# zixunh/vipe

Measured on AMD Instinct MI355X. Metric: dense-BA+flow update iters/s, 512x384 48-KF graph, higher is better.
Workload: dtype f16 (correlation, GRU; fp32 accumulate) + f32 geometry/BA (fp64 reduced system)

## Files before the change

### include/vipe_amd.h

```cpp
#ifndef VIPE_AMD_H
#define VIPE_AMD_H

#include <stdint.h>

#ifdef __cplusplus
extern "C" {
#endif

#define VIPE_F16 0
#define VIPE_F32 1
#define VIPE_F64 2
#define VIPE_U8 3

#define VIPE_OK 0
#define VIPE_EINVAL (-1)
#define VIPE_ENOSPACE (-2)
#define VIPE_EUNSUPPORTED (-3)

#define VIPE_PYRAMID_REFERENCE 0
#define VIPE_PYRAMID_BLOCKED 1

#define VIPE_CAM_PINHOLE 0
#define VIPE_CAM_MEI 1
#define VIPE_CAM_PANORAMA 2
// ... 225 lines not shown
                                 int64_t Lv, int heads, int C, int L, int64_t Lq, int P, int dtype, void* stream);

#define VIPE_ACT_NONE 0
#define VIPE_ACT_RELU 1
#define VIPE_ACT_SIGMOID 2
#define VIPE_ACT_TANH 3
int vipe_conv_pack_weights(const void* d_w_oihw, void* d_w_packed, int Cout, int Cin, int KH, int KW, int src_dtype,
                           void* stream);
int vipe_conv2d_nhwc_f16(const void* d_x, const void* d_w_packed, const float* d_bias, const float* d_extra,
                         void* d_y, int B, int H, int W, int Cin, int cin_total, int cin_off, int Cout,
                         int cout_total, int cout_off, int KH, int KW, int act, void* stream);

int vipe_conv_packed_dims(int Cout, int Cin, int KH, int KW, int* cout_pad, int* cin_pad, int* k_pad);

#define VIPE_CONV_PARTIAL 6
#define VIPE_CONV_ACCINIT_F32 0x100
int vipe_conv2d_fused(const void* d_x0, int x0_ctot, int x0_coff, const void* d_x1, int x1_ctot, int x1_coff,
                      int split, const void* d_w_packed, const float* d_bias, const float* d_extra, int extra_stride,
                      int extra_off, void* d_y, int y_ctot, int y_coff, void* d_y2, int y2_ctot, int y2_coff,
                      const void* d_net, int net_ctot, int net_coff, const void* d_z, float* d_fout,
                      const void* d_accinit, int ai_ctot, int ai_coff, int B, int H, int W, int Cin, int Cout, int KH,
                      int KW, int act, int mode, void* stream);

typedef struct {
  const void *corr0_w, *corr2_w, *flow0_w, *flow2_w, *gw_w, *zr_w, *q_w, *zr_s_w, *q_s_w, *heads0_w, *heads2_w, *agg2_w, *eta_w;
  const void *zr_n_w, *zr_x_w;
  const float *corr0_b, *corr2_b, *flow0_b, *flow2_b, *gw_b, *zr_b, *q_b, *heads0_b, *heads2_b, *agg2_b, *eta_b;
  const float* glo_wT;
  const float* glo_b;
} vipe_update_weights;
typedef struct {
  int E, H, W, n_src;
  const void* levels[4];
  const float* coords;
  const int* slots;
  int h2, w2, pyramid_layout;
  const void* corr;
  const void* motn;
  const void* net;
  void* net_out;
  void* xbuf;
  const void* pgate;
  void *c1, *f1, *zb, *rnet;
  void* hbuf;
  float* dw;
  float *glo, *extra;
  const int *order, *rowptr;
  void *agg, *a2;
  float* eta;
  void* side_stream;
  float* pzr;
  int gate_state;
} vipe_update_buffers;
int vipe_update_operator(const vipe_update_weights* weights, const vipe_update_buffers* buffers, void* stream);

int vipe_update_gate_state(const vipe_update_weights* weights, const vipe_update_buffers* buffers, const void* d_net,
                           int parts, void* stream);
typedef struct {
  const vipe_update_weights* weights;
  const vipe_update_buffers* buffers;
  const void* net;
  const int* bounds;
  int n_bounds;
} vipe_gate_state_job;
int vipe_update_gate_state_piece(void* user, int piece, int n_pieces, void* stream);

int vipe_glo_context(const float* d_glo_sum, const float* d_wT, const float* d_bias, float* d_extra, int E, int hw,
// ... 93 lines not shown
```

### vipe_amd/csrc/conv_mfma.hip

```cpp
#include <stdlib.h>

#include <type_traits>

#include "common.cuh"

namespace {

typedef _Float16 half8 __attribute__((ext_vector_type(8)));
typedef _Float16 half4 __attribute__((ext_vector_type(4)));
typedef float float16v __attribute__((ext_vector_type(16)));
typedef float float4v __attribute__((ext_vector_type(4)));

enum Epi { EPI_PLAIN = 0, EPI_GLO = 1, EPI_ZR = 2, EPI_Q = 3, EPI_HEADS = 4, EPI_ETA = 5, EPI_PARTIAL = 6 };

struct ConvArgs {
  const half_t* x0; int x0_ctot, x0_coff;
  const half_t* x1; int x1_ctot, x1_coff;
  int split;
  const half_t* w;
  const float* bias;
  const float* extra;
  int extra_stride, extra_off;
  half_t* y; int y_ctot, y_coff;
  int B, H, W, Cin, Cin_pad, Cout, Cout_pad, KH, KW, nsteps;
  int act, epi;
  const half_t* net; int net_ctot, net_coff;
  const half_t* zbuf;
  half_t* y2; int y2_ctot, y2_coff;
  float* fout;
  const half_t* accinit; int ai_ctot, ai_coff;
  int ai_f32;
  int f_wp, f_hwp, f_tiles, f_pieces, f_xbytes, f_p1lo, f_p1hi;
  unsigned f_magic;
};

constexpr int BNP = 128;
constexpr int BK = 64;

__device__ __forceinline__ int swz(int row, int k8) { return row * 128 + ((k8 ^ ((row >> 1) & 7)) << 4); }

__device__ __forceinline__ float act_apply(float v, int act) {
  switch (act) {
    case VIPE_ACT_RELU: return fmaxf(v, 0.0f);
    case VIPE_ACT_SIGMOID: return 1.0f / (1.0f + __expf(-v));
    case VIPE_ACT_TANH: return tanhf(v);
    default: return v;
// ... 316 lines not shown

constexpr int H32_PIECES = (HALO_ROWS + 15) / 16;
constexpr int H32_XBYTES = H32_PIECES * 1024;
constexpr int H32_XP = (H32_PIECES + 7) / 8;
constexpr int H32_BK = 32;

__device__ __forceinline__ int swzf(int row) { return ((row >> 2) & 1) << 1; }
__device__ __forceinline__ int swz32(int row, int c) { return row * 64 + ((c ^ swzf(row)) << 4); }


__device__ __forceinline__ int flat_pixel(int q, int e, int H, int W, int wp, int hwp, unsigned magic) {
  if ((unsigned)q >= (unsigned)hwp) return -1;
  const int y = (int)__umulhi((unsigned)q, magic);
  const int x = q - y * wp;
  return x < W ? (e * H + y) * W + x : -1;
}

template <int BMC, int KS, bool M16, int VAR = 0, bool FLAT = false>
__global__ __launch_bounds__(512) __attribute__((amdgpu_waves_per_eu(4, 4))) void conv_halo32_kernel(ConvArgs a, int gy) {
  static_assert(M16, "only the 16x16x32 form exists");
  constexpr int MI = BMC >= 128 ? 4 : 2, NJ = BMC == 32 ? 2 : 4;
  constexpr int BP = HALO_TH * HALO_TW;
  constexpr int WSTAGE = BMC * 64;
  extern __shared__ __align__(16) unsigned char lds[];

  const int tid = threadIdx.x, lane = tid & 63, wave = __builtin_amdgcn_readfirstlane(tid >> 6);
  const int wm = BMC == 32 ? 0 : (wave >> 2), wn = wave & 3;
  const int pxh = BMC == 32 ? (wave >> 2) * 32 : 0;
  const int L = xcd_remap(blockIdx.x, gridDim.x);
  const int tile = L / gy, cout0 = (L % gy) * BMC;
// ... 207 lines not shown
#pragma unroll
        for (int j = 0; j < NJ; ++j) {
          const int64_t m = pix_of(wn * 64 + j * 16 + l16);
          if (FLAT && m < 0) continue;
#pragma unroll
          for (int i = 0; i < MI; ++i) {
            const int cg = cout0 + wm * (MI * 16) + i * 16 + 4 * lk;
            if (cg + 4 <= a.Cout)
              *reinterpret_cast<float4*>(a.fout + m * a.y_ctot + a.y_coff + cg) =
                  make_float4(acc16[i][j][0], acc16[i][j][1], acc16[i][j][2], acc16[i][j][3]);
          }
        }
        return;
      }
    }
    constexpr int PITCH = BMC + 8;
    half_t* stage = reinterpret_cast<half_t*>(lds);
    auto stage_all = [&](auto ACTC) {
      constexpr int ACT = decltype(ACTC)::value;
      auto put = [&](int cl, int pl, float4 b, float v0, float v1, float v2, float v3) {
        half4 h;
        h[0] = (half_t)act_apply(v0 + b.x, ACT);
        h[1] = (half_t)act_apply(v1 + b.y, ACT);
        h[2] = (half_t)act_apply(v2 + b.z, ACT);
        h[3] = (half_t)act_apply(v3 + b.w, ACT);
        *reinterpret_cast<half4*>(stage + pl * PITCH + cl) = h;
      };
      auto bias4 = [&](int cl) {
        const int cg = cout0 + cl;
        float4 b = *reinterpret_cast<const float4*>(a.bias + cg);
// ... 477 lines not shown
  VIPE_CHECK_ARG(d_w_oihw && d_w_packed);
  VIPE_CHECK_ARG(src_dtype == VIPE_F16 || src_dtype == VIPE_F32);
  int cp, cinp, kp;
  if (vipe_conv_packed_dims(Cout, Cin, KH, KW, &cp, &cinp, &kp) != VIPE_OK) return VIPE_EINVAL;
  VIPE_CHECK_ARG(Cin == 4 || Cin % 8 == 0);
  const int64_t total = (int64_t)kp * cp;
  pack_weights_kernel<<<(int)std::min<int64_t>((total + 255) / 256, 4096), 256, 0, as_stream(stream)>>>(
      d_w_oihw, (half_t*)d_w_packed, Cout, Cin, KH, KW, cp, cinp, kp, src_dtype == VIPE_F32, Cin == 4);
  return vipe_launch_status();
}

}

namespace {

template <typename K>
void allow_lds(K kernel, std::atomic<uint64_t>& seen, size_t bytes) {
  vipe_once_per_device(seen, [&] { (void)hipFuncSetAttribute((const void*)kernel, hipFuncAttributeMaxDynamicSharedMemorySize, (int)bytes); });
}
constexpr size_t MAX_LDS = 160 * 1024;

bool flat_geometry(ConvArgs& a, int pad) {
  a.f_wp = a.W + pad;
  a.f_hwp = a.H * a.f_wp;
  a.f_tiles = (a.f_hwp + 255) / 256;
  a.f_magic = (unsigned)(((1ull << 32) + (unsigned)a.f_wp - 1) / (unsigned)a.f_wp);
  const int rows = 256 + 2 * a.f_wp + 2;
  a.f_pieces = (rows + 15) / 16;
  a.f_xbytes = a.f_pieces * 1024;
  a.f_p1lo = (a.f_wp + 1) / 16;
  a.f_p1hi = (a.f_wp + 256) / 16;
  return a.f_wp >= 2 && a.f_pieces <= 8 * H32_XP && a.f_hwp < (1 << 23);
}

inline bool needs_tile_kernel(const ConvArgs& a) { return a.accinit || a.epi == EPI_PARTIAL || a.ai_f32; }

template <int BMC, int KS, int VAR, bool FLAT>
int launch_halo32(const ConvArgs& a, int tiles, int gy, size_t lds, hipStream_t s) {
  static std::atomic<uint64_t> seen{0};
  allow_lds(conv_halo32_kernel<BMC, KS, true, VAR, FLAT>, seen, FLAT ? MAX_LDS : lds);
  conv_halo32_kernel<BMC, KS, true, VAR, FLAT><<<dim3(tiles * gy), 512, lds, s>>>(a, gy);
  return vipe_launch_status();
}

template <bool FLAT>
int launch_halo_family(ConvArgs& a, int cp, int64_t M, hipStream_t s) {
  const bool split_ok = a.split >= a.Cin || a.split % H32_BK == 0;
  const int tiles = FLAT ? a.B * a.f_tiles : (int)(M / (HALO_TH * HALO_TW));
  const size_t xb = FLAT ? (size_t)a.f_xbytes : (size_t)H32_XBYTES;
  if (needs_tile_kernel(a)) {
    const bool ok = cp >= 64 && split_ok && !(a.KH == 3 && a.Cout <= 16) && !(a.epi == EPI_PARTIAL && a.Cout % 4 != 0) &&
                    !(a.ai_f32 && !a.accinit);
    if (!ok) return VIPE_EUNSUPPORTED;
  }
  if (a.KH == 3 && a.Cout <= 16 && cp == 32 && split_ok && (a.epi == EPI_HEADS || a.epi == EPI_ETA || a.epi == EPI_PLAIN)) {
    static std::atomic<uint64_t> seen{0};
    const size_t lds = 2 * NRW_WBYTES + 2 * xb + 1024;
    allow_lds(conv_halo32_narrow_kernel<FLAT>, seen, FLAT ? MAX_LDS : lds);
    conv_halo32_narrow_kernel<FLAT><<<dim3(tiles), 512, lds, s>>>(a);
    return vipe_launch_status();
  }
  if (!split_ok) return VIPE_EUNSUPPORTED;
  const int bmc = cp >= 128 ? 128 : cp;
  const int gy = cp >= 128 ? cp / 128 : 1;
// ... 119 lines not shown
                                  int y_coff, void* d_y2, int y2_ctot, int y2_coff, const void* d_net, int net_ctot,
                                  int net_coff, const void* d_z, float* d_fout, const void* d_accinit, int ai_ctot,
                                  int ai_coff, int B, int H, int W, int Cin, int Cout, int KH, int KW, int act, int mode,
                                  void* stream) {
  VIPE_CHECK_ARG(d_x0 && d_w_packed && d_bias);
  VIPE_CHECK_ARG(!d_accinit || (ai_ctot % 4 == 0 && ai_coff % 4 == 0 && ai_coff + Cout <= ai_ctot));
  VIPE_CHECK_ARG(B >= 0 && H > 0 && W > 0 && Cin > 0 && Cout > 0 && (KH & 1) && (KW & 1));
  if (Cin == 4) {
    VIPE_CHECK_ARG(split >= Cin && x0_ctot % 4 == 0 && x0_coff % 4 == 0);
  } else {
    VIPE_CHECK_ARG(Cin % 8 == 0 && x0_ctot % 8 == 0 && x0_coff % 8 == 0);
    VIPE_CHECK_ARG(split >= Cin || (split % 64 == 0 && d_x1 && x1_ctot % 8 == 0 && x1_coff % 8 == 0));
  }
  const int ai_f32 = (mode & VIPE_CONV_ACCINIT_F32) != 0;
  mode &= ~VIPE_CONV_ACCINIT_F32;
  VIPE_CHECK_ARG(mode >= EPI_PLAIN && mode <= EPI_PARTIAL);
  if (mode == EPI_PARTIAL) VIPE_CHECK_ARG(d_fout && y_ctot % 4 == 0 && y_coff % 4 == 0 && y_coff + Cout <= y_ctot && !d_extra);
  if (mode == EPI_PLAIN) VIPE_CHECK_ARG(d_y && y_ctot % 4 == 0 && y_coff % 4 == 0);
  if (mode == EPI_GLO) VIPE_CHECK_ARG(d_net && d_fout);
  if (mode == EPI_ZR) VIPE_CHECK_ARG(d_y && d_y2 && d_net && Cout == 256);
  if (mode == EPI_Q) VIPE_CHECK_ARG(d_y && d_net && d_z && Cout == 128);
  if (mode == EPI_HEADS) VIPE_CHECK_ARG(d_fout && Cout == 4);
  if (mode == EPI_ETA) VIPE_CHECK_ARG(d_fout && Cout == 1);
  ConvArgs a = {};
  a.x0 = (const half_t*)d_x0; a.x0_ctot = x0_ctot; a.x0_coff = x0_coff;
  a.x1 = (const half_t*)(d_x1 ? d_x1 : d_x0); a.x1_ctot = d_x1 ? x1_ctot : x0_ctot; a.x1_coff = d_x1 ? x1_coff : x0_coff;
  a.split = split > Cin ? Cin : split;
  a.w = (const half_t*)d_w_packed; a.bias = d_bias; a.extra = d_extra; a.extra_stride = extra_stride; a.extra_off = extra_off;
  a.y = (half_t*)d_y; a.y_ctot = y_ctot; a.y_coff = y_coff;
  a.y2 = (half_t*)d_y2; a.y2_ctot = y2_ctot; a.y2_coff = y2_coff;
  a.net = (const half_t*)d_net; a.net_ctot = net_ctot; a.net_coff = net_coff;
  a.zbuf = (const half_t*)d_z; a.fout = d_fout;
  a.accinit = (const half_t*)d_accinit; a.ai_ctot = ai_ctot; a.ai_coff = ai_coff; a.ai_f32 = ai_f32;
  a.B = B; a.H = H; a.W = W; a.Cin = Cin; a.Cout = Cout; a.KH = KH; a.KW = KW;
  a.act = act; a.epi = mode;
  return launch_conv(a, as_stream(stream));
}

}
```

### vipe_amd/csrc/update_op.hip

```cpp
#include "common.cuh"

namespace {

__global__ __launch_bounds__(384) void glo_gemm_kernel(const float* __restrict__ glo, const float* __restrict__ wT ,
                                                       const float* __restrict__ b, float* __restrict__ extra, float inv_hw) {
  __shared__ float g[128];
  const int e = blockIdx.x, t = threadIdx.x;
  if (t < 128) g[t] = glo[(int64_t)e * 128 + t] * inv_hw;
  __syncthreads();
  float acc = b[t];
#pragma unroll 8
  for (int k = 0; k < 128; ++k) acc = __builtin_fmaf(g[k], wT[k * 384 + t], acc);
  extra[(int64_t)e * 384 + t] = acc;
}

__global__ __launch_bounds__(256) void update_finish_kernel(const float* __restrict__ coords1, const float* __restrict__ dw,
                                                            const unsigned char* __restrict__ mask, float* __restrict__ target,
                                                            float* __restrict__ weight, const float* __restrict__ eta,
                                                            const int64_t* __restrict__ du, float* __restrict__ damping,
                                                            int64_t n_px, int64_t n_eta, int P) {
  const int64_t i = (int64_t)blockIdx.x * 256 + threadIdx.x;
  if (i < n_px) {
    const float2 c = reinterpret_cast<const float2*>(coords1)[i];
    const float4 d = reinterpret_cast<const float4*>(dw)[i];
// ... 84 lines not shown
                          nullptr, 0, 0, b->net, 128, 0, b->zb, nullptr, b->pgate, 384, 256, E, H, W, 320, 128, 3, 3,
                          VIPE_ACT_NONE, 3, stream));
  } else if (b->pgate) {
    RUN(vipe_conv2d_fused(b->net, 128, 0, b->xbuf, 320, 128, 128, wt->zr_s_w, wt->zr_b, b->extra, 384, 0, b->zb, 128, 0, b->rnet,
                          128, 0, b->net, 128, 0, nullptr, nullptr, b->pgate, 384, 0, E, H, W, 320, 256, 3, 3, VIPE_ACT_NONE, 2,
                          stream));
    RUN(vipe_conv2d_fused(b->rnet, 128, 0, b->xbuf, 320, 128, 128, wt->q_s_w, wt->q_b, b->extra, 384, 256, b->net_out, 128, 0,
                          nullptr, 0, 0, b->net, 128, 0, b->zb, nullptr, b->pgate, 384, 256, E, H, W, 320, 128, 3, 3,
                          VIPE_ACT_NONE, 3, stream));
  } else {
    RUN(vipe_conv2d_fused(b->net, 128, 0, b->xbuf, 320, 0, 128, wt->zr_w, wt->zr_b, b->extra, 384, 0, b->zb, 128, 0, b->rnet, 128,
                          0, b->net, 128, 0, nullptr, nullptr, nullptr, 0, 0, E, H, W, 448, 256, 3, 3, VIPE_ACT_NONE, 2, stream));
    RUN(vipe_conv2d_fused(b->rnet, 128, 0, b->xbuf, 320, 0, 128, wt->q_w, wt->q_b, b->extra, 384, 256, b->net_out, 128, 0, nullptr,
                          0, 0, b->net, 128, 0, b->zb, nullptr, nullptr, 0, 0, E, H, W, 448, 128, 3, 3, VIPE_ACT_NONE, 3, stream));
  }
  RUN(vipe_conv2d_fused(b->net_out, 128, 0, nullptr, 0, 0, 128, wt->heads0_w, wt->heads0_b, nullptr, 0, 0, b->hbuf, 384, 0,
                        nullptr, 0, 0, nullptr, 0, 0, nullptr, nullptr, nullptr, 0, 0, E, H, W, 128, 384, 3, 3, VIPE_ACT_RELU, 0,
                        stream));
  const bool two_tails = s2 && b->n_src > 0;
  if (two_tails) FORK(2);
  RUN(vipe_conv2d_fused(b->hbuf, 384, 0, nullptr, 0, 0, 256, wt->heads2_w, wt->heads2_b, nullptr, 0, 0, nullptr, 0, 0, nullptr, 0,
                        0, nullptr, 0, 0, nullptr, b->dw, nullptr, 0, 0, E, H, W, 256, 4, 3, 3, VIPE_ACT_NONE, 4,
                        two_tails ? stream2 : stream));
  if (b->n_src > 0) {
    VIPE_CHECK_ARG(b->order && b->rowptr && b->agg && b->a2 && b->eta);
    RUN(vipe_segment_mean_nhwc_f16(b->hbuf, 384, 256, b->order, b->rowptr, b->agg, b->n_src, (int64_t)H * W, 128, stream));
    RUN(vipe_conv2d_fused(b->agg, 128, 0, nullptr, 0, 0, 128, wt->agg2_w, wt->agg2_b, nullptr, 0, 0, b->a2, 128, 0, nullptr, 0, 0,
                          nullptr, 0, 0, nullptr, nullptr, nullptr, 0, 0, b->n_src, H, W, 128, 128, 3, 3, VIPE_ACT_RELU, 0,
                          stream));
    RUN(vipe_conv2d_fused(b->a2, 128, 0, nullptr, 0, 0, 128, wt->eta_w, wt->eta_b, nullptr, 0, 0, nullptr, 0, 0, nullptr, 0, 0,
                          nullptr, 0, 0, nullptr, b->eta, nullptr, 0, 0, b->n_src, H, W, 128, 1, 3, 3, VIPE_ACT_NONE, 5, stream));
  }
  if (two_tails) JOIN(3);
#undef FORK
#undef JOIN
#undef RUN
  return vipe_launch_status();
}

VIPE_EXPORT int vipe_update_gate_state(const vipe_update_weights* wt, const vipe_update_buffers* b, const void* d_net,
                                       int parts, void* stream) {
  VIPE_CHECK_ARG(wt && b && b->E >= 0 && b->H > 0 && b->W > 0 && parts >= 1 && parts <= 3);
  if (b->E == 0) return VIPE_OK;
  VIPE_CHECK_ARG(d_net && (!(parts & 1) || (b->glo && b->extra)) && (!(parts & 2) || (b->pgate && b->pzr && wt->zr_n_w)));
  const int E = b->E, H = b->H, W = b->W;
  hipStream_t s = as_stream(stream);
// ... 62 lines not shown
```

### vipe_amd/slam/update_engine.py

```python

import ctypes
import os

import torch

from .._lib import check, lib, parse_struct, ptr, stream_ptr

UpdateWeights = parse_struct("vipe_update_weights")
UpdateBuffers = parse_struct("vipe_update_buffers")
GateStateJob = parse_struct("vipe_gate_state_job")

ACT = {"none": 0, "relu": 1, "sigmoid": 2, "tanh": 3}
EPI = {"plain": 0, "glo": 1, "zr": 2, "q": 3, "heads": 4, "eta": 5, "partial": 6}
ACCINIT_F32 = 0x100
CORR_CH = 200


class _Packed:

    def __init__(self, w_oihw, bias, device):
        w = w_oihw.detach().to(device=device, dtype=torch.float16).contiguous()
        self.cout, self.cin, self.kh, self.kw = w.shape
        cp, cinp, kp = ctypes.c_int(), ctypes.c_int(), ctypes.c_int()
        check(lib().vipe_conv_packed_dims(self.cout, self.cin, self.kh, self.kw, ctypes.addressof(cp),
                                          ctypes.addressof(cinp), ctypes.addressof(kp)), "conv_packed_dims")
        self.packed = torch.empty(kp.value * cp.value, dtype=torch.float16, device=device)
        check(lib().vipe_conv_pack_weights(ptr(w), ptr(self.packed), self.cout, self.cin, self.kh, self.kw, 0,
                                           stream_ptr(w)), "conv_pack_weights")
        assert bias.numel() == self.cout, (tuple(bias.shape), self.cout)
        self.bias = torch.zeros(cp.value, dtype=torch.float32, device=device)
        self.bias[:self.cout] = bias.detach().to(device=device, dtype=torch.float32).reshape(-1)
        self.flops_per_pixel = 2.0 * self.cout * self.cin * self.kh * self.kw


def segment_csr(ix, n_src):
    order = torch.argsort(ix, stable=True).to(torch.int32).contiguous()
    counts = torch.bincount(ix, minlength=n_src)
    rowptr = torch.zeros(n_src + 1, dtype=torch.int32, device=ix.device)
    rowptr[1:] = torch.cumsum(counts, 0).to(torch.int32)
    return order, rowptr


class UpdateEngine:
    def __init__(self, module, device):
        self.device = device
        self.m = module
        self._bufs = {}
# ... 19 lines not shown
        wz, bz = wb(m.gru.convz)
        wr, br = wb(m.gru.convr)
        self.zr = _Packed(torch.cat([wz, wr], 0), torch.cat([bz, br], 0), d)
        wq, bq = wb(m.gru.convq)
        self.q = _Packed(wq, bq, d)
        rest = list(range(0, 128)) + list(range(256, 448))
        self.zr_s = _Packed(torch.cat([wz, wr], 0)[:, rest].contiguous(), torch.cat([bz, br], 0), d)
        self.q_s = _Packed(wq[:, rest].contiguous(), bq, d)
        self.gates_inp = _Packed(torch.cat([wz, wr, wq], 0)[:, 128:256].contiguous(), torch.zeros(384, device=d), d)
        self.zr_n = _Packed(torch.cat([wz, wr], 0)[:, 0:128].contiguous(), torch.cat([bz, br], 0), d)
        self.zr_x = _Packed(torch.cat([wz, wr], 0)[:, 256:448].contiguous(), torch.cat([bz, br], 0), d)
        wd0, bd0 = wb(m.delta[0])
        ww0, bw0 = wb(m.weight[0])
        wa1, ba1 = wb(m.agg.conv1)
        self.heads0 = _Packed(torch.cat([wd0, ww0, wa1], 0), torch.cat([bd0, bw0, ba1], 0), d)
        wd2, bd2 = wb(m.delta[2])
        ww2, bw2 = wb(m.weight[2])
        h2 = torch.zeros(4, 256, 3, 3, device=d, dtype=f16)
        h2[0:2, 0:128] = wd2[:2]
        h2[2:4, 128:256] = ww2[:2]
        self.heads2 = _Packed(h2, torch.cat([bd2[:2], bw2[:2]], 0), d)
        self.agg2 = _Packed(*wb(m.agg.conv2), d)
        self.eta = _Packed(*wb(m.agg.eta[0]), d)
        self.upmask = _Packed(*wb(m.agg.upmask[0]), d)
        g = m.gru
        self.glo_w = torch.cat([g.convz_glo.weight, g.convr_glo.weight, g.convq_glo.weight], 0).detach().to(d).float() \
            .reshape(384, 128).t().contiguous()
        self.glo_b = torch.cat([g.convz_glo.bias, g.convr_glo.bias, g.convq_glo.bias], 0).detach().to(d).float()
        wd_ = UpdateWeights()
        for name, pk in dict(corr0=self.corr0, corr2=self.corr2, flow0=self.flow0, flow2=self.flow2, gw=self.gw, zr=self.zr,
                             q=self.q, heads0=self.heads0, heads2=self.heads2, agg2=self.agg2, eta=self.eta).items():
            setattr(wd_, name + "_w", pk.packed.data_ptr())
            setattr(wd_, name + "_b", pk.bias.data_ptr())
        wd_.zr_s_w, wd_.q_s_w = self.zr_s.packed.data_ptr(), self.q_s.packed.data_ptr()
        wd_.zr_n_w, wd_.zr_x_w = self.zr_n.packed.data_ptr(), self.zr_x.packed.data_ptr()
        wd_.glo_wT, wd_.glo_b = self.glo_w.data_ptr(), self.glo_b.data_ptr()
        self._wdesc = wd_
        self._bdesc = {}

    def _conv(self, pk, x0, x0_coff, B, H, W, y=None, y_coff=0, act="none", mode="plain", x1=None, x1_coff=0,
              split=None, extra=None, extra_off=0, y2=None, y2_coff=0, net=None, net_coff=0, z=None, fout=None,
              cin=None, accinit=None, ai_coff=0):
        cin = pk.cin if cin is None else cin
        split = cin if split is None else split
        check(lib().vipe_conv2d_fused(
            ptr(x0), x0.shape[-1], x0_coff, ptr(x1), x1.shape[-1] if x1 is not None else 0, x1_coff, split,
            ptr(pk.packed), ptr(pk.bias), ptr(extra), extra.shape[-1] if extra is not None else 0, extra_off,
            ptr(y), (y if y is not None else fout).shape[-1] if (y is not None or mode == "partial") else 0, y_coff,
            ptr(y2), y2.shape[-1] if y2 is not None else 0, y2_coff,
            ptr(net), net.shape[-1] if net is not None else 0, net_coff, ptr(z), ptr(fout), ptr(accinit),
            accinit.shape[-1] if accinit is not None else 0, ai_coff, B, H, W, cin, pk.cout,
# ... 56 lines not shown
            cum, acc = [0], 0.0
            for f in fractions[:-1]:
                acc += f
                cum.append(min(E, int(round(E * acc / sum(fractions)))))
            cum.append(E)
            bounds = (ctypes.c_int * len(cum))(*cum)
            job.bounds, job.n_bounds = ctypes.addressof(bounds), len(cum)
        fn = ctypes.cast(lib().vipe_update_gate_state_piece, ctypes.c_void_p).value
        gs = dict(net_ptr=net.data_ptr(), pgate_ptr=pgate.data_ptr(), shape=tuple(net.shape), pzr=pzr, extra=extra,
                  n_staged=E, keep=(b, job, bounds), gen=self._gate_gen)
        return gs, (lambda stream: (stream.cuda_stream, fn, ctypes.addressof(job)))

    def gate_state_matches(self, gs, net, pgate):
        return (gs is not None and pgate is not None and gs["net_ptr"] == net.data_ptr() and
                gs["pgate_ptr"] == pgate.data_ptr() and gs["shape"] == tuple(net.shape) and gs.get("gen") == self._gate_gen)

    def _buf(self, name, shape, dtype=torch.float16):
        t = self._bufs.get(name)
        if t is None or tuple(t.shape) != tuple(shape) or t.dtype != dtype:
            t = torch.empty(shape, dtype=dtype, device=self.device)
            self._bufs[name] = t
        return t

    @torch.no_grad()
    def forward_nhwc(self, net, xbuf, corr, motn, ix=None, n_src=None, net_out=None, want_upmask=False, csr=None,
                     pgate=None, native=True, gate_state=None):
        E, H, W, _ = net.shape
        if not self.gate_state_matches(gate_state, net, pgate):
            gate_state = None
        if gate_state is None:
# ... 32 lines not shown
                       accinit=gate_state["pzr"], ai_coff=0, cin=192)
            if Es < E:
                self._conv(self.zr_s, net[Es:], 0, E - Es, H, W, x1=xbuf[Es:], x1_coff=128, split=128, y=zb[Es:], y2=rnet[Es:],
                           net=net[Es:], mode="zr", extra=extra[Es:], accinit=pgate[Es:], ai_coff=0)
            self._conv(self.q_s, rnet, 0, E, H, W, x1=xbuf, x1_coff=128, split=128, y=net_out, net=net, z=zb, mode="q",
                       extra=extra, extra_off=256, accinit=pgate, ai_coff=256)
        elif pgate is not None:
            self._conv(self.zr_s, net, 0, E, H, W, x1=xbuf, x1_coff=128, split=128, y=zb, y2=rnet, net=net, mode="zr",
                       extra=extra, accinit=pgate, ai_coff=0)
            self._conv(self.q_s, rnet, 0, E, H, W, x1=xbuf, x1_coff=128, split=128, y=net_out, net=net, z=zb, mode="q",
                       extra=extra, extra_off=256, accinit=pgate, ai_coff=256)
        else:
            self._conv(self.zr, net, 0, E, H, W, x1=xbuf, split=128, y=zb, y2=rnet, net=net, mode="zr", extra=extra)
            self._conv(self.q, rnet, 0, E, H, W, x1=xbuf, split=128, y=net_out, net=net, z=zb, mode="q", extra=extra,
                       extra_off=256)
        self._conv(self.heads0, net_out, 0, E, H, W, y=hbuf, act="relu")
        self._conv(self.heads2, hbuf, 0, E, H, W, mode="heads", fout=dw, cin=256)
        eta = upmask = None
        if ix is not None:
            if n_src is None:
                n_src = int(ix.max().item()) + 1 if ix.numel() else 0
            if csr is None:
                csr = segment_csr(ix, n_src)
            order, rowptr = csr
            agg = self._buf("agg", (n_src, H, W, 128))
            check(lib().vipe_segment_mean_nhwc_f16(ptr(hbuf), 384, 256, ptr(order), ptr(rowptr), ptr(agg), n_src, H * W,
                                                   128, stream_ptr(hbuf)), "segment_mean")
            a2 = self._buf("a2", (n_src, H, W, 128))
            eta = self._buf("eta", (n_src, H, W), torch.float32)
            self._conv(self.agg2, agg, 0, n_src, H, W, y=a2, act="relu")
            self._conv(self.eta, a2, 0, n_src, H, W, mode="eta", fout=eta)
            if want_upmask:
                upmask = torch.empty((n_src, H, W, 576), dtype=torch.float16, device=self.device)
                self._conv(self.upmask, a2, 0, n_src, H, W, y=upmask)
        return net_out, dw, eta, upmask

    def _forward_native(self, net, xbuf, corr, motn, ix, n_src, net_out, want_upmask, csr, pgate, scratch,
                        gate_state=None):
        c1, f1, zb, rnet, hbuf, dw, glo = scratch
        E, H, W, _ = net.shape
        extra = self._buf("extra", (E, 384), torch.float32)
        eta = agg = a2 = order = rowptr = None
        if ix is not None:
            if n_src is None:
                n_src = int(ix.max().item()) + 1 if ix.numel() else 0
            if csr is None:
                csr = segment_csr(ix, n_src)
            order, rowptr = csr
            agg = self._buf("agg", (n_src, H, W, 128))
            a2 = self._buf("a2", (n_src, H, W, 128))
            eta = self._buf("eta", (n_src, H, W), torch.float32)
        lookup = isinstance(corr, tuple)
        tensors = (net, net_out, xbuf, motn, pgate, c1, f1, zb, rnet, hbuf, dw, glo, extra, order, rowptr, agg, a2, eta) + \
            ((tuple(corr[1]) + (corr[2],) + ((corr[3],) if len(corr) > 3 and corr[3] is not None else ())) if lookup else (corr,))
        pzr = gate_state["pzr"] if gate_state is not None else None
        two_streams = E >= self.op_side_min_edges
        if two_streams and self._op_side is None:
            self._op_side = torch.cuda.Stream(device=self.device)
        key = tuple(0 if t is None else t.data_ptr() for t in tensors) + (E, H, W, n_src or 0, two_streams,
                                                                         0 if pzr is None else pzr.data_ptr(),
                                                                         0 if pzr is None else int(gate_state["n_staged"]))
        b = self._bdesc.get(key)
        if b is None:
            if len(self._bdesc) > 16:
                self._bdesc.clear()
            b = UpdateBuffers()
            b.E, b.H, b.W, b.n_src = E, H, W, int(n_src or 0) if ix is not None else 0
            if lookup:
                lv = corr[1]
                for i in range(4):
                    b.levels[i] = lv[i].data_ptr()
                b.coords = corr[2].data_ptr()
                b.slots = corr[3].data_ptr() if len(corr) > 3 and corr[3] is not None else None
                if len(corr) > 4 and corr[4] is not None:
                    b.h2, b.w2 = int(corr[4][0]), int(corr[4][1])
                else:
                    b.h2, b.w2 = int(lv[2].shape[3]) << 2, int(lv[2].shape[4]) << 2
                b.pyramid_layout = 1 if lv[0].dim() == 7 else 0
            else:
                b.corr = corr.data_ptr()
            for name, t in dict(motn=motn, net=net, net_out=net_out, xbuf=xbuf, pgate=pgate, c1=c1, f1=f1, zb=zb, rnet=rnet,
                                hbuf=hbuf, dw=dw, glo=glo, extra=extra, order=order, rowptr=rowptr, agg=agg, a2=a2,
                                eta=eta).items():
                setattr(b, name, None if t is None else t.data_ptr())
            if pzr is not None:
                b.pzr, b.gate_state = pzr.data_ptr(), int(gate_state["n_staged"])
            if two_streams:
                b.side_stream = self._op_side.cuda_stream
            self._bdesc[key] = b
        check(lib().vipe_update_operator(ctypes.addressof(self._wdesc), ctypes.addressof(b), stream_ptr(net)),
              "update_operator")
        upmask = None
        if want_upmask and ix is not None:
            upmask = torch.empty((n_src, H, W, 576), dtype=torch.float16, device=self.device)
            self._conv(self.upmask, a2, 0, n_src, H, W, y=upmask)
        return net_out, dw, eta, upmask

    @torch.no_grad()
# ... 28 lines not shown
```

Measured before the change: 263.0.

## Fuse heads 3x3 conv into heads0 epilogue and split agg branch per consumer

Splits the heads0 conv by consumer. The agg1 slice is computed first so the aggregation chain can fork onto the side stream early. The delta/weight 256-channel slice now runs a new fused epilogue: it applies the 4-output heads2 3x3 conv in registers and LDS via MFMA, writes interior pixels directly, and writes halo contributions to a border buffer. A small finish kernel adds neighbour-tile border sums, bias and sigmoid. This removes the hbuf round-trip and a separate heads2 launch, at the cost of extra LDS use, an extra kernel and a more complex epilogue.

```diff
diff --git a/include/vipe_amd.h b/include/vipe_amd.h
--- a/include/vipe_amd.h
+++ b/include/vipe_amd.h
@@ -263,6 +263,7 @@
 int vipe_conv_packed_dims(int Cout, int Cin, int KH, int KW, int* cout_pad, int* cin_pad, int* k_pad);
 
 #define VIPE_CONV_PARTIAL 6
+#define VIPE_CONV_HEADS_FUSED 7
 #define VIPE_CONV_ACCINIT_F32 0x100
 int vipe_conv2d_fused(const void* d_x0, int x0_ctot, int x0_coff, const void* d_x1, int x1_ctot, int x1_coff,
                       int split, const void* d_w_packed, const float* d_bias, const float* d_extra, int extra_stride,
@@ -271,12 +272,19 @@
                       const void* d_accinit, int ai_ctot, int ai_coff, int B, int H, int W, int Cin, int Cout, int KH,
                       int KW, int act, int mode, void* stream);
 
+int vipe_heads_fused_ok(int H, int W);
+int vipe_heads_border_floats(int E, int H, int W, int64_t* n_floats);
+int vipe_heads_finish(float* d_dw, const float* d_border, const float* d_bias, int E, int H, int W, void* stream);
+
 typedef struct {
   const void *corr0_w, *corr2_w, *flow0_w, *flow2_w, *gw_w, *zr_w, *q_w, *zr_s_w, *q_s_w, *heads0_w, *heads2_w, *agg2_w, *eta_w;
   const void *zr_n_w, *zr_x_w;
   const float *corr0_b, *corr2_b, *flow0_b, *flow2_b, *gw_b, *zr_b, *q_b, *heads0_b, *heads2_b, *agg2_b, *eta_b;
   const float* glo_wT;
   const float* glo_b;
+  const void *agg1_w, *heads_dw_w;
+  const float *agg1_b, *heads_dw_b;
+  const void* heads2_frag;
 } vipe_update_weights;
 typedef struct {
   int E, H, W, n_src;
@@ -300,6 +308,7 @@
   void* side_stream;
   float* pzr;
   int gate_state;
+  float* hborder;
 } vipe_update_buffers;
 int vipe_update_operator(const vipe_update_weights* weights, const vipe_update_buffers* buffers, void* stream);
 
diff --git a/vipe_amd/csrc/conv_mfma.hip b/vipe_amd/csrc/conv_mfma.hip
--- a/vipe_amd/csrc/conv_mfma.hip
+++ b/vipe_amd/csrc/conv_mfma.hip
@@ -11,7 +11,7 @@
 typedef float float16v __attribute__((ext_vector_type(16)));
 typedef float float4v __attribute__((ext_vector_type(4)));
 
-enum Epi { EPI_PLAIN = 0, EPI_GLO = 1, EPI_ZR = 2, EPI_Q = 3, EPI_HEADS = 4, EPI_ETA = 5, EPI_PARTIAL = 6 };
+enum Epi { EPI_PLAIN = 0, EPI_GLO = 1, EPI_ZR = 2, EPI_Q = 3, EPI_HEADS = 4, EPI_ETA = 5, EPI_PARTIAL = 6, EPI_HEADS_FUSED = 7 };
 
 struct ConvArgs {
   const half_t* x0; int x0_ctot, x0_coff;
@@ -30,6 +30,8 @@
   float* fout;
   const half_t* accinit; int ai_ctot, ai_coff;
   int ai_f32;
+  const half_t* w2;
+  float* border;
   int f_wp, f_hwp, f_tiles, f_pieces, f_xbytes, f_p1lo, f_p1hi;
   unsigned f_magic;
 };
@@ -376,6 +378,12 @@
   const int y = (int)__umulhi((unsigned)q, magic);
   const int x = q - y * wp;
   return x < W ? (e * H + y) * W + x : -1;
+}
+
+constexpr int HB_N = 2 * (HALO_TW + 2) + 2 * HALO_TH;
+constexpr int HG_PITCH = HALO_TH * HALO_TW + 4;
+__host__ __device__ __forceinline__ int hb_index(int py, int px) {
+  return py < 0 ? px + 1 : py >= HALO_TH ? (HALO_TW + 2) + px + 1 : px < 0 ? 2 * (HALO_TW + 2) + py : 2 * (HALO_TW + 2) + HALO_TH + py;
 }
 
 template <int BMC, int KS, bool M16, int VAR = 0, bool FLAT = false>
@@ -613,6 +621,61 @@
         return;
       }
     }
+    if constexpr (VAR == 3) {
+      static_assert(BMC == 128 && KS == 3 && !FLAT, "the fused heads exist for the aligned 128-cout 3x3 tile only");
+      const int slice = cout0 >> 7;
+      float* G = reinterpret_cast<float*>(lds);
+      float4 bq[MI];
+#pragma unroll
+      for (int i = 0; i < MI; ++i) bq[i] = *reinterpret_cast<const float4*>(a.bias + cout0 + wm * 64 + i * 16 + 4 * lk);
+      const half8* af = reinterpret_cast<const half8*>(a.w2) + (slice * 2 + wm) * 4 * 64 + lane;
+      half8 afr[2][2];
+#pragma unroll
+      for (int q = 0; q < 4; ++q) afr[q >> 1][q & 1] = af[q * 64];
+#pragma unroll
+      for (int j = 0; j < NJ; ++j) {
+        half8 hb[2];
+#pragma unroll
+        for (int i = 0; i < MI; ++i) {
+          hb[i >> 1][(i & 1) * 4 + 0] = (half_t)fmaxf(acc16[i][j][0] + bq[i].x, 0.0f);
+          hb[i >> 1][(i & 1) * 4 + 1] = (half_t)fmaxf(acc16[i][j][1] + bq[i].y, 0.0f);
+          hb[i >> 1][(i & 1) * 4 + 2] = (half_t)fmaxf(acc16[i][j][2] + bq[i].z, 0.0f);
+          hb[i >> 1][(i & 1) * 4 + 3] = (half_t)fmaxf(acc16[i][j][3] + bq[i].w, 0.0f);
+        }
+        float4v g0 = float4v{0.0f, 0.0f, 0.0f, 0.0f}, g1 = g0;
+        g0 = __builtin_amdgcn_mfma_f32_16x16x32_f16(afr[0][0], hb[0], g0, 0, 0, 0);
+        g0 = __builtin_amdgcn_mfma_f32_16x16x32_f16(afr[0][1], hb[1], g0, 0, 0, 0);
+        g1 = __builtin_amdgcn_mfma_f32_16x16x32_f16(afr[1][0], hb[0], g1, 0, 0, 0);
+        g1 = __builtin_amdgcn_mfma_f32_16x16x32_f16(afr[1][1], hb[1], g1, 0, 0, 0);
+        const int p = wn * 64 + j * 16 + l16;
+#pragma unroll
+        for (int r = 0; r < 4; ++r) G[(wm * 18 + 4 * lk + r) * HG_PITCH + p] = g0[r];
+        if (lk == 0) {
+          G[(wm * 18 + 16) * HG_PITCH + p] = g1[0];
+          G[(wm * 18 + 17) * HG_PITCH + p] = g1[1];
+        }
+      }
+      __syncthreads();
+      for (int idx = tid; idx < 6 * 66 * 2; idx += 512) {
+        const int o = idx & 1, pos = idx >> 1, py = pos / 66 - 1, px = pos % 66 - 1;
+        const int yy = y0 + py, xx = x0 + px;
+        if (yy < 0 || yy >= a.H || xx < 0 || xx >= a.W) continue;
+        float sum = 0.0f;
+#pragma unroll
+        for (int tap = 0; tap < 9; ++tap) {
+          const int sy = py + tap / 3 - 1, sx = px + tap % 3 - 1;
+          if ((unsigned)sy < (unsigned)HALO_TH && (unsigned)sx < (unsigned)HALO_TW) {
+            const float* gp = G + (tap * 2 + o) * HG_PITCH + sy * HALO_TW + sx;
+            sum += gp[0] + gp[18 * HG_PITCH];
+          }
+        }
+        if ((unsigned)py < (unsigned)HALO_TH && (unsigned)px < (unsigned)HALO_TW)
+          a.fout[((int64_t)(e * a.H + yy) * a.W + xx) * 4 + slice * 2 + o] = sum;
+        else
+          a.border[((int64_t)tile * HB_N + hb_index(py, px)) * 4 + slice * 2 + o] = sum;
+      }
+      return;
+    }
     constexpr int PITCH = BMC + 8;
     half_t* stage = reinterpret_cast<half_t*>(lds);
     auto stage_all = [&](auto ACTC) {
@@ -1120,6 +1183,35 @@
 
 namespace {
 
+__global__ __launch_bounds__(256) void heads_finish_kernel(float* __restrict__ dw, const float* __restrict__ border,
+                                                           const float* __restrict__ bias, int64_t M, int H, int W) {
+  const int64_t m = (int64_t)blockIdx.x * 256 + threadIdx.x;
+  if (m >= M) return;
+  const int x = (int)(m % W), y = (int)((m / W) % H), e = (int)(m / ((int64_t)W * H));
+  const int xsegs = W / HALO_TW, ysegs = H / HALO_TH;
+  const int ty = y / HALO_TH, tx = x / HALO_TW, py = y % HALO_TH, px = x % HALO_TW;
+  const int tile = (e * ysegs + ty) * xsegs + tx;
+  float4 s = reinterpret_cast<const float4*>(dw)[m];
+  auto add = [&](int t, int bi) {
+    const float4 v = reinterpret_cast<const float4*>(border)[(int64_t)t * HB_N + bi];
+    s.x += v.x; s.y += v.y; s.z += v.z; s.w += v.w;
+  };
+  const bool up = py == 0 && ty > 0, down = py == HALO_TH - 1 && ty < ysegs - 1;
+  const bool left = px == 0 && tx > 0, right = px == HALO_TW - 1 && tx < xsegs - 1;
+  if (up) add(tile - xsegs, hb_index(HALO_TH, px));
+  if (down) add(tile + xsegs, hb_index(-1, px));
+  if (left) add(tile - 1, hb_index(py, HALO_TW));
+  if (right) add(tile + 1, hb_index(py, -1));
+  if (up && left) add(tile - xsegs - 1, hb_index(HALO_TH, HALO_TW));
+  if (up && right) add(tile - xsegs + 1, hb_index(HALO_TH, -1));
+  if (down && left) add(tile + xsegs - 1, hb_index(-1, HALO_TW));
+  if (down && right) add(tile + xsegs + 1, hb_index(-1, -1));
+  const float4 b = *reinterpret_cast<const float4*>(bias);
+  const float v0 = s.x + b.x, v1 = s.y + b.y, v2 = s.z + b.z, v3 = s.w + b.w;
+  reinterpret_cast<float4*>(dw)[m] = make_float4((float)(half_t)v0, (float)(half_t)v1, (float)(half_t)act_apply(v2, VIPE_ACT_SIGMOID),
+                                                 (float)(half_t)act_apply(v3, VIPE_ACT_SIGMOID));
+}
+
 template <typename K>
 void allow_lds(K kernel, std::atomic<uint64_t>& seen, size_t bytes) {
   vipe_once_per_device(seen, [&] { (void)hipFuncSetAttribute((const void*)kernel, hipFuncAttributeMaxDynamicSharedMemorySize, (int)bytes); });
@@ -1139,7 +1231,7 @@
   return a.f_wp >= 2 && a.f_pieces <= 8 * H32_XP && a.f_hwp < (1 << 23);
 }
 
-inline bool needs_tile_kernel(const ConvArgs& a) { return a.accinit || a.epi == EPI_PARTIAL || a.ai_f32; }
+inline bool needs_tile_kernel(const ConvArgs& a) { return a.accinit || a.epi == EPI_PARTIAL || a.ai_f32 || a.epi == EPI_HEADS_FUSED; }
 
 template <int BMC, int KS, int VAR, bool FLAT>
 int launch_halo32(const ConvArgs& a, int tiles, int gy, size_t lds, hipStream_t s) {
@@ -1154,6 +1246,10 @@
   const bool split_ok = a.split >= a.Cin || a.split % H32_BK == 0;
   const int tiles = FLAT ? a.B * a.f_tiles : (int)(M / (HALO_TH * HALO_TW));
   const size_t xb = FLAT ? (size_t)a.f_xbytes : (size_t)H32_XBYTES;
+  if (a.epi == EPI_HEADS_FUSED) {
+    if constexpr (FLAT) return VIPE_EUNSUPPORTED;
+    else return launch_halo32<128, 3, 3, false>(a, tiles, 2, 3 * (size_t)128 * 64 + 2 * xb + 1024, s);
+  }
   if (needs_tile_kernel(a)) {
     const bool ok = cp >= 64 && split_ok && !(a.KH == 3 && a.Cout <= 16) && !(a.epi == EPI_PARTIAL && a.Cout % 4 != 0) &&
                     !(a.ai_f32 && !a.accinit);
@@ -1303,7 +1399,12 @@
   }
   const int ai_f32 = (mode & VIPE_CONV_ACCINIT_F32) != 0;
   mode &= ~VIPE_CONV_ACCINIT_F32;
-  VIPE_CHECK_ARG(mode >= EPI_PLAIN && mode <= EPI_PARTIAL);
+  VIPE_CHECK_ARG(mode >= EPI_PLAIN && mode <= EPI_HEADS_FUSED);
+  if (mode == EPI_HEADS_FUSED) {
+    VIPE_CHECK_ARG(d_fout && d_net && d_y2 && Cin == 128 && Cout == 256 && KH == 3 && KW == 3 && act == VIPE_ACT_RELU &&
+                   !d_extra && !d_accinit && !ai_f32 && split >= Cin);
+    if (H % HALO_TH != 0 || W % HALO_TW != 0) return VIPE_EUNSUPPORTED;
+  }
   if (mode == EPI_PARTIAL) VIPE_CHECK_ARG(d_fout && y_ctot % 4 == 0 && y_coff % 4 == 0 && y_coff + Cout <= y_ctot && !d_extra);
   if (mode == EPI_PLAIN) VIPE_CHECK_ARG(d_y && y_ctot % 4 == 0 && y_coff % 4 == 0);
   if (mode == EPI_GLO) VIPE_CHECK_ARG(d_net && d_fout);
@@ -1318,6 +1419,10 @@
   a.w = (const half_t*)d_w_packed; a.bias = d_bias; a.extra = d_extra; a.extra_stride = extra_stride; a.extra_off = extra_off;
   a.y = (half_t*)d_y; a.y_ctot = y_ctot; a.y_coff = y_coff;
   a.y2 = (half_t*)d_y2; a.y2_ctot = y2_ctot; a.y2_coff = y2_coff;
+  if (mode == EPI_HEADS_FUSED) {
+    a.w2 = (const half_t*)d_net; a.border = (float*)d_y2;
+    d_net = nullptr; a.y2 = nullptr;
+  }
   a.net = (const half_t*)d_net; a.net_ctot = net_ctot; a.net_coff = net_coff;
   a.zbuf = (const half_t*)d_z; a.fout = d_fout;
   a.accinit = (const half_t*)d_accinit; a.ai_ctot = ai_ctot; a.ai_coff = ai_coff; a.ai_f32 = ai_f32;
@@ -1326,4 +1431,25 @@
   return launch_conv(a, as_stream(stream));
 }
 
-}
+VIPE_EXPORT int vipe_heads_fused_ok(int H, int W) {
+  const char* v = getenv("VIPE_AMD_FUSED_HEADS");
+  const bool enabled = !(v && v[0] == '0');
+  return enabled && H > 0 && W > 0 && H % HALO_TH == 0 && W % HALO_TW == 0;
+}
+
+VIPE_EXPORT int vipe_heads_border_floats(int E, int H, int W, int64_t* n) {
+  VIPE_CHECK_ARG(n && E >= 0 && H > 0 && W > 0 && H % HALO_TH == 0 && W % HALO_TW == 0);
+  *n = (int64_t)E * (H / HALO_TH) * (W / HALO_TW) * HB_N * 4;
+  return VIPE_OK;
+}
+
+VIPE_EXPORT int vipe_heads_finish(float* d_dw, const float* d_border, const float* d_bias, int E, int H, int W, void* stream) {
+  VIPE_CHECK_ARG(E >= 0 && H > 0 && W > 0 && H % HALO_TH == 0 && W % HALO_TW == 0);
+  if (E == 0) return VIPE_OK;
+  VIPE_CHECK_ARG(d_dw && d_border && d_bias);
+  const int64_t M = (int64_t)E * H * W;
+  heads_finish_kernel<<<(unsigned)((M + 255) / 256), 256, 0, as_stream(stream)>>>(d_dw, d_border, d_bias, M, H, W);
+  return vipe_launch_status();
+}
+
+}
diff --git a/vipe_amd/csrc/update_op.hip b/vipe_amd/csrc/update_op.hip
--- a/vipe_amd/csrc/update_op.hip
+++ b/vipe_amd/csrc/update_op.hip
@@ -122,22 +122,43 @@
     RUN(vipe_conv2d_fused(b->rnet, 128, 0, b->xbuf, 320, 0, 128, wt->q_w, wt->q_b, b->extra, 384, 256, b->net_out, 128, 0, nullptr,
                           0, 0, b->net, 128, 0, b->zb, nullptr, nullptr, 0, 0, E, H, W, 448, 128, 3, 3, VIPE_ACT_NONE, 3, stream));
   }
-  RUN(vipe_conv2d_fused(b->net_out, 128, 0, nullptr, 0, 0, 128, wt->heads0_w, wt->heads0_b, nullptr, 0, 0, b->hbuf, 384, 0,
-                        nullptr, 0, 0, nullptr, 0, 0, nullptr, nullptr, nullptr, 0, 0, E, H, W, 128, 384, 3, 3, VIPE_ACT_RELU, 0,
-                        stream));
   const bool two_tails = s2 && b->n_src > 0;
-  if (two_tails) FORK(2);
-  RUN(vipe_conv2d_fused(b->hbuf, 384, 0, nullptr, 0, 0, 256, wt->heads2_w, wt->heads2_b, nullptr, 0, 0, nullptr, 0, 0, nullptr, 0,
-                        0, nullptr, 0, 0, nullptr, b->dw, nullptr, 0, 0, E, H, W, 256, 4, 3, 3, VIPE_ACT_NONE, 4,
-                        two_tails ? stream2 : stream));
-  if (b->n_src > 0) {
+  const bool by_consumer = wt->agg1_w && wt->agg1_b && wt->heads_dw_w && wt->heads_dw_b;
+  auto heads0 = [&](const void* w, const float* bias, int coff, int cout) -> int {
+    return vipe_conv2d_fused(b->net_out, 128, 0, nullptr, 0, 0, 128, w, bias, nullptr, 0, 0, b->hbuf, 384, coff, nullptr, 0, 0,
+                             nullptr, 0, 0, nullptr, nullptr, nullptr, 0, 0, E, H, W, 128, cout, 3, 3, VIPE_ACT_RELU, 0, stream);
+  };
+  auto agg_chain = [&](void* st) -> int {
+    if (b->n_src <= 0) return VIPE_OK;
     VIPE_CHECK_ARG(b->order && b->rowptr && b->agg && b->a2 && b->eta);
-    RUN(vipe_segment_mean_nhwc_f16(b->hbuf, 384, 256, b->order, b->rowptr, b->agg, b->n_src, (int64_t)H * W, 128, stream));
+    RUN(vipe_segment_mean_nhwc_f16(b->hbuf, 384, 256, b->order, b->rowptr, b->agg, b->n_src, (int64_t)H * W, 128, st));
     RUN(vipe_conv2d_fused(b->agg, 128, 0, nullptr, 0, 0, 128, wt->agg2_w, wt->agg2_b, nullptr, 0, 0, b->a2, 128, 0, nullptr, 0, 0,
-                          nullptr, 0, 0, nullptr, nullptr, nullptr, 0, 0, b->n_src, H, W, 128, 128, 3, 3, VIPE_ACT_RELU, 0,
-                          stream));
-    RUN(vipe_conv2d_fused(b->a2, 128, 0, nullptr, 0, 0, 128, wt->eta_w, wt->eta_b, nullptr, 0, 0, nullptr, 0, 0, nullptr, 0, 0,
-                          nullptr, 0, 0, nullptr, b->eta, nullptr, 0, 0, b->n_src, H, W, 128, 1, 3, 3, VIPE_ACT_NONE, 5, stream));
+                          nullptr, 0, 0, nullptr, nullptr, nullptr, 0, 0, b->n_src, H, W, 128, 128, 3, 3, VIPE_ACT_RELU, 0, st));
+    return vipe_conv2d_fused(b->a2, 128, 0, nullptr, 0, 0, 128, wt->eta_w, wt->eta_b, nullptr, 0, 0, nullptr, 0, 0, nullptr, 0, 0,
+                             nullptr, 0, 0, nullptr, b->eta, nullptr, 0, 0, b->n_src, H, W, 128, 1, 3, 3, VIPE_ACT_NONE, 5, st);
+  };
+  auto heads2 = [&](void* st) -> int {
+    return vipe_conv2d_fused(b->hbuf, 384, 0, nullptr, 0, 0, 256, wt->heads2_w, wt->heads2_b, nullptr, 0, 0, nullptr, 0, 0,
+                             nullptr, 0, 0, nullptr, 0, 0, nullptr, b->dw, nullptr, 0, 0, E, H, W, 256, 4, 3, 3, VIPE_ACT_NONE, 4, st);
+  };
+  if (by_consumer && two_tails) {
+    RUN(heads0(wt->agg1_w, wt->agg1_b, 256, 128));
+    FORK(2);
+    RUN(agg_chain(stream2));
+    if (wt->heads2_frag && b->hborder && vipe_heads_fused_ok(H, W)) {
+      RUN(vipe_conv2d_fused(b->net_out, 128, 0, nullptr, 0, 0, 128, wt->heads_dw_w, wt->heads_dw_b, nullptr, 0, 0, nullptr, 0, 0,
+                            b->hborder, 0, 0, wt->heads2_frag, 0, 0, nullptr, b->dw, nullptr, 0, 0, E, H, W, 128, 256, 3, 3,
+                            VIPE_ACT_RELU, VIPE_CONV_HEADS_FUSED, stream));
+      RUN(vipe_heads_finish(b->dw, b->hborder, wt->heads2_b, E, H, W, stream));
+    } else {
+      RUN(heads0(wt->heads_dw_w, wt->heads_dw_b, 0, 256));
+      RUN(heads2(stream));
+    }
+  } else {
+    RUN(heads0(wt->heads0_w, wt->heads0_b, 0, 384));
+    if (two_tails) FORK(2);
+    RUN(heads2(two_tails ? stream2 : stream));
+    RUN(agg_chain(stream));
   }
   if (two_tails) JOIN(3);
 #undef FORK
diff --git a/vipe_amd/slam/update_engine.py b/vipe_amd/slam/update_engine.py
--- a/vipe_amd/slam/update_engine.py
+++ b/vipe_amd/slam/update_engine.py
@@ -11,7 +11,7 @@
 GateStateJob = parse_struct("vipe_gate_state_job")
 
 ACT = {"none": 0, "relu": 1, "sigmoid": 2, "tanh": 3}
-EPI = {"plain": 0, "glo": 1, "zr": 2, "q": 3, "heads": 4, "eta": 5, "partial": 6}
+EPI = {"plain": 0, "glo": 1, "zr": 2, "q": 3, "heads": 4, "eta": 5, "partial": 6, "heads_fused": 7}
 ACCINIT_F32 = 0x100
 CORR_CH = 200
 
@@ -31,6 +31,22 @@
         self.bias = torch.zeros(cp.value, dtype=torch.float32, device=device)
         self.bias[:self.cout] = bias.detach().to(device=device, dtype=torch.float32).reshape(-1)
         self.flops_per_pixel = 2.0 * self.cout * self.cin * self.kh * self.kw
+
+
+def heads2_fragment_index():
+    import numpy as np
+    s, h, rb, ip, lane, e = np.meshgrid(*[np.arange(n) for n in (2, 2, 2, 2, 64, 8)], indexing="ij")
+    row = 16 * rb + lane % 16
+    tap, o = row // 2, row % 2
+    ch = 128 * s + 64 * h + 16 * (2 * ip + e // 4) + 4 * (lane // 16) + e % 4
+    valid = row < 18
+    return np.where(valid, 2 * s + o, 0), ch, np.where(valid, tap, 0), valid
+
+
+def pack_heads2_fragments(h2_oihw):
+    out, ch, tap, valid = (torch.from_numpy(a).to(h2_oihw.device) for a in heads2_fragment_index())
+    w = h2_oihw.reshape(4, 256, 9)[out, ch, tap]
+    return torch.where(valid, w, torch.zeros_like(w)).to(torch.float16).contiguous().reshape(-1)
 
 
 def segment_csr(ix, n_src):
@@ -80,12 +96,17 @@
         ww0, bw0 = wb(m.weight[0])
         wa1, ba1 = wb(m.agg.conv1)
         self.heads0 = _Packed(torch.cat([wd0, ww0, wa1], 0), torch.cat([bd0, bw0, ba1], 0), d)
+        self.heads_by_consumer = os.environ.get("VIPE_AMD_HEADS_BY_CONSUMER", "1") != "0"
+        self.agg1 = _Packed(wa1, ba1, d)
+        self.heads_dw = _Packed(torch.cat([wd0, ww0], 0), torch.cat([bd0, bw0], 0), d)
         wd2, bd2 = wb(m.delta[2])
         ww2, bw2 = wb(m.weight[2])
         h2 = torch.zeros(4, 256, 3, 3, device=d, dtype=f16)
         h2[0:2, 0:128] = wd2[:2]
         h2[2:4, 128:256] = ww2[:2]
         self.heads2 = _Packed(h2, torch.cat([bd2[:2], bw2[:2]], 0), d)
+        self.heads2_frag = pack_heads2_fragments(h2)
+        self.fused_heads_on = self.heads_by_consumer and os.environ.get("VIPE_AMD_FUSED_HEADS", "1") != "0"
         self.agg2 = _Packed(*wb(m.agg.conv2), d)
         self.eta = _Packed(*wb(m.agg.eta[0]), d)
         self.upmask = _Packed(*wb(m.agg.upmask[0]), d)
@@ -101,6 +122,11 @@
         wd_.zr_s_w, wd_.q_s_w = self.zr_s.packed.data_ptr(), self.q_s.packed.data_ptr()
         wd_.zr_n_w, wd_.zr_x_w = self.zr_n.packed.data_ptr(), self.zr_x.packed.data_ptr()
         wd_.glo_wT, wd_.glo_b = self.glo_w.data_ptr(), self.glo_b.data_ptr()
+        if self.heads_by_consumer:
+            wd_.agg1_w, wd_.agg1_b = self.agg1.packed.data_ptr(), self.agg1.bias.data_ptr()
+            wd_.heads_dw_w, wd_.heads_dw_b = self.heads_dw.packed.data_ptr(), self.heads_dw.bias.data_ptr()
+            if self.fused_heads_on:
+                wd_.heads2_frag = self.heads2_frag.data_ptr()
         self._wdesc = wd_
         self._bdesc = {}
 
@@ -187,6 +213,14 @@
     def gate_state_matches(self, gs, net, pgate):
         return (gs is not None and pgate is not None and gs["net_ptr"] == net.data_ptr() and
                 gs["pgate_ptr"] == pgate.data_ptr() and gs["shape"] == tuple(net.shape) and gs.get("gen") == self._gate_gen)
+
+    def fused_heads(self, H, W):
+        return self.fused_heads_on and bool(lib().vipe_heads_fused_ok(H, W))
+
+    def _hborder(self, E, H, W):
+        n = ctypes.c_int64()
+        check(lib().vipe_heads_border_floats(E, H, W, ctypes.addressof(n)), "heads_border_floats")
+        return self._buf("hborder", (n.value,), torch.float32)
 
     def _buf(self, name, shape, dtype=torch.float16):
         t = self._bufs.get(name)
@@ -249,15 +283,12 @@
             self._conv(self.zr, net, 0, E, H, W, x1=xbuf, split=128, y=zb, y2=rnet, net=net, mode="zr", extra=extra)
             self._conv(self.q, rnet, 0, E, H, W, x1=xbuf, split=128, y=net_out, net=net, z=zb, mode="q", extra=extra,
                        extra_off=256)
-        self._conv(self.heads0, net_out, 0, E, H, W, y=hbuf, act="relu")
-        self._conv(self.heads2, hbuf, 0, E, H, W, mode="heads", fout=dw, cin=256)
-        eta = upmask = None
-        if ix is not None:
-            if n_src is None:
-                n_src = int(ix.max().item()) + 1 if ix.numel() else 0
-            if csr is None:
-                csr = segment_csr(ix, n_src)
-            order, rowptr = csr
+        if n_src is None and ix is not None:
+            n_src = int(ix.max().item()) + 1 if ix.numel() else 0
+        eta = upmask = a2 = None
+
+        def agg_chain():
+            order, rowptr = csr if csr is not None else segment_csr(ix, n_src)
             agg = self._buf("agg", (n_src, H, W, 128))
             check(lib().vipe_segment_mean_nhwc_f16(ptr(hbuf), 384, 256, ptr(order), ptr(rowptr), ptr(agg), n_src, H * W,
                                                    128, stream_ptr(hbuf)), "segment_mean")
@@ -265,9 +296,29 @@
             eta = self._buf("eta", (n_src, H, W), torch.float32)
             self._conv(self.agg2, agg, 0, n_src, H, W, y=a2, act="relu")
             self._conv(self.eta, a2, 0, n_src, H, W, mode="eta", fout=eta)
-            if want_upmask:
-                upmask = torch.empty((n_src, H, W, 576), dtype=torch.float16, device=self.device)
-                self._conv(self.upmask, a2, 0, n_src, H, W, y=upmask)
+            return a2, eta
+
+        chain = ix is not None and n_src > 0
+        if self.heads_by_consumer and chain and E >= self.op_side_min_edges:
+            self._conv(self.agg1, net_out, 0, E, H, W, y=hbuf, y_coff=256, act="relu")
+            a2, eta = agg_chain()
+            if self.fused_heads(H, W):
+                hborder = self._hborder(E, H, W)
+                self._conv(self.heads_dw, net_out, 0, E, H, W, act="relu", mode="heads_fused", net=self.heads2_frag,
+                           y2=hborder, fout=dw)
+                check(lib().vipe_heads_finish(ptr(dw), ptr(hborder), ptr(self.heads2.bias), E, H, W, stream_ptr(dw)),
+                      "heads_finish")
+            else:
+                self._conv(self.heads_dw, net_out, 0, E, H, W, y=hbuf, act="relu")
+                self._conv(self.heads2, hbuf, 0, E, H, W, mode="heads", fout=dw, cin=256)
+        else:
+            self._conv(self.heads0, net_out, 0, E, H, W, y=hbuf, act="relu")
+            self._conv(self.heads2, hbuf, 0, E, H, W, mode="heads", fout=dw, cin=256)
+            if ix is not None:
+                a2, eta = agg_chain()
+        if ix is not None and want_upmask:
+            upmask = torch.empty((n_src, H, W, 576), dtype=torch.float16, device=self.device)
+            self._conv(self.upmask, a2, 0, n_src, H, W, y=upmask)
         return net_out, dw, eta, upmask
 
     def _forward_native(self, net, xbuf, corr, motn, ix, n_src, net_out, want_upmask, csr, pgate, scratch,
@@ -286,7 +337,9 @@
             a2 = self._buf("a2", (n_src, H, W, 128))
             eta = self._buf("eta", (n_src, H, W), torch.float32)
         lookup = isinstance(corr, tuple)
-        tensors = (net, net_out, xbuf, motn, pgate, c1, f1, zb, rnet, hbuf, dw, glo, extra, order, rowptr, agg, a2, eta) + \
+        hborder = self._hborder(E, H, W) if self.fused_heads(H, W) else None
+        tensors = (net, net_out, xbuf, motn, pgate, c1, f1, zb, rnet, hbuf, dw, glo, extra, order, rowptr, agg, a2, eta,
+                   hborder) + \
             ((tuple(corr[1]) + (corr[2],) + ((corr[3],) if len(corr) > 3 and corr[3] is not None else ())) if lookup else (corr,))
         pzr = gate_state["pzr"] if gate_state is not None else None
         two_streams = E >= self.op_side_min_edges
@@ -316,7 +369,7 @@
                 b.corr = corr.data_ptr()
             for name, t in dict(motn=motn, net=net, net_out=net_out, xbuf=xbuf, pgate=pgate, c1=c1, f1=f1, zb=zb, rnet=rnet,
                                 hbuf=hbuf, dw=dw, glo=glo, extra=extra, order=order, rowptr=rowptr, agg=agg, a2=a2,
-                                eta=eta).items():
+                                eta=eta, hborder=hborder).items():
                 setattr(b, name, None if t is None else t.data_ptr())
             if pzr is not None:
                 b.pzr, b.gate_state = pzr.data_ptr(), int(gate_state["n_staged"])
```

Result: faster. 273.5, median of 6 (+4.0%).
